# acproject/wsi-segmentation-pipeline

Hardware: AMD Instinct MI355X
Metric: patches/sec (256×256×3) whole-slide inference, 1/2/4/8 MI355X + CPU ref (higher is better)
Workload: dtype fp16 + MX-fp6 cross terms (fp32 accumulate); 1 GPU; cfg3: ONE 40000x40000 synthetic slide, tile 256 stride 256 -> 24648 tiles sharded over 1 rank(s) (each holds only its own slide regions: 4.80 GB on rank 0), ResNet-18 trunk + Classifier, fused read+normalise+conv HIP path, 1 all-gather, float64 stitch + softmax; tiles_total=24648, batch=6200, mode=mx, parallelism=tile-shard x1 + 1 all-gather, batches_in_flight=2

## Files before the change

### include/wsi_hip.h

```cpp
#ifndef WSI_HIP_H
#define WSI_HIP_H
#include <stddef.h>
#include <stdint.h>

#ifdef __cplusplus
extern "C" {
#endif

#define WSI_HIP_ABI_VERSION 8
int wsi_hip_abi_version(void);

size_t wsi_pf_bytes(int n, int h, int w, int c, int planes);
long long wsi_pf_pixel_index(int n, int y, int x, int h, int w);

size_t wsi_prepack_conv_bytes(int cout, int cin, int k, int planes);
int wsi_prepack_conv(const float* w, const float* bn_weight, const float* bn_bias, const float* bn_mean,
                     const float* bn_var, float eps, int cout, int cin, int k, int planes, void* wpk_out,
                     float* bias_out);
size_t wsi_prepack_stem_bytes(int planes);
int wsi_prepack_stem(const float* w, const float* bn_weight, const float* bn_bias, const float* bn_mean,
                     const float* bn_var, float eps, int planes, void* wpk_out, float* bias_out);
int wsi_prepack_stem_u8(const float* w, const float* bn_weight, const float* bn_bias, const float* bn_mean,
                        const float* bn_var, float eps, const float mean[3], const float std_[3], int planes,
                        void* wpk_out, float* bias_out);
// ... 6 lines not shown
                                     const float* stem_bias_u8, const float* norm_mean_std ,
                                     int n, int h, int w, float* scratch, void* out_pf, int planes, void* stream);

int wsi_stem_conv7x7_bn_relu_maxpool_lines96(const float* in_f32, const uint8_t* slide, long long slide_pitch_bytes,
                                             int slide_h, int slide_w, const int* tile_xy, const float* lut,
                                             const void* stem_wpk, const float* stem_bias, const void* stem_wpk_u8,
                                             const float* stem_bias_u8, const float* norm_mean_std, int n, int h, int w,
                                             float* scratch, void* out_pf96, long long plane96, void* stream);

enum {
    WSI_STEM_MODE_UNFUSED = 0,
    WSI_STEM_MODE_FUSED = 1,
    WSI_STEM_MODE_FUSED_LUT = 2,
    WSI_STEM_MODE_FUSED_ONE_STRIP = 3,
    WSI_STEM_MODE_FUSED_STRIPS = 4
};
int wsi_stem_set_mode(int fused, int rows_per_seg);

int wsi_conv3x3_bn_act(const void* in_pf, void* out_pf, const void* resid_pf, const void* wpk, const float* bias,
                       int n, int h_in, int w_in, int cin, int cout, int stride, int relu, int planes,
                       void* stream);
int wsi_conv1x1_bn(const void* in_pf, void* out_pf, const void* wpk, const float* bias, int n, int h_in, int w_in,
                   int cin, int cout, int stride, int planes, void* stream);
int wsi_conv3x3_up_concat_bn_act(const void* up_pf, const void* skip_pf, void* out_pf, const void* wpk, const float* bias, int n, int h, int w,
                                 int c_up, int c_skip, int cout, int relu, int planes, void* stream);
int wsi_conv3x3s2_ds_fused(const void* in_pf, void* out_conv_pf, void* out_ds_pf, const void* wpk3, const float* bias3,
                           const void* wpk1, const float* bias1, int n, int h_in, int w_in, int cin, int cout, int planes,
                           void* stream);
int wsi_s2_slab_images(int n, int h_in, int w_in, int cin, int planes);
size_t wsi_pf_split_bytes(int n, int h, int w, int c, int planes);
int wsi_conv3x3_bn_act_split(const void* in_pf, void* out_split, const void* resid_pf, const void* wpk, const float* bias,
                             int n, int h, int w, int cin, int cout, int relu, int planes, void* stream);
int wsi_conv3x3s2_ds_fused_split(const void* in_split, void* out_conv_pf, void* out_ds_pf, const void* wpk3,
                                 const float* bias3, const void* wpk1, const float* bias1, int n, int h_in, int w_in,
                                 int cin, int cout, int planes, void* stream);
enum {
    WSI_CONV_MODE_S2_GATHER = 0,
    WSI_CONV_MODE_S2_SLAB = 1,
    WSI_CONV_MODE_S2_SLAB_128 = 3,
    WSI_CONV_MODE_XCD_ORDER = 8,
    WSI_CONV_MODE_WIDE_FROM_256 = 16,
    WSI_CONV_MODE_WIDE_NEVER = 32,
    WSI_CONV_MODE_S2_ABLATE = 64,
    WSI_CONV_MODE_NO_S2_SPLIT = 128,
    WSI_CONV_MODE_XCD_RANGES_OFF = 256,
    WSI_CONV_MODE_XCD_RANGES_L1 = 512,
    WSI_CONV_MODE_L1_SLAB3 = 1024,
    WSI_CONV_MODE_NO_DS_FOLD = 2048,
    WSI_CONV_MODE_NO_SLAB_PAIR = 4096,
    WSI_CONV_MODE_L1_LINES128 = 16384,
    WSI_CONV_MODE_S2_NT2 = 32768,
    WSI_CONV_MODE_UNET_CONCAT_PASS = 65536,
    WSI_CONV_MODE_WIDE_NO_D8 = 131072,
    WSI_CONV_MODE_L1_PERSISTENT = 1048576,
    WSI_CONV_MODE_UNET_NO_TAIL = 2097152,
    WSI_CONV_MODE_UNET_TAIL_FORM1 = 4194304,
    WSI_CONV_MODE_UNET_X0_UNFUSED = 8388608
};
int wsi_conv_set_mode(int mode);
int wsi_conv3x3_bn_act_cfg(const void* in_pf, void* out_pf, const void* resid_pf, const void* wpk, const float* bias,
                           int n, int h_in, int w_in, int cin, int cout, int stride, int relu, int planes, int cfg,
                           void* stream);

int wsi_avgpool_fc(const void* in_pf, int n, int h, int w, int c, const float* fc_w, const float* fc_b, int k,
                   float* feat_out, float* logits_out, int planes, void* stream);
int wsi_linear(const float* x, const float* w, const float* bias, float* y, int b, int k, int j, int relu,
               void* stream);

int wsi_pf_pack(const float* in_nchw, void* out_pf, int n, int c, int h, int w, int planes, void* stream);
int wsi_pf_unpack(const void* in_pf, float* out_nchw, int n, int c, int h, int w, int planes, void* stream);

typedef struct {
    const void* stem_w;   const float* stem_b;
    const void* stem_w_u8; const float* stem_b_u8;
    float norm[6];
    const void* conv_w[16]; const float* conv_b[16];
    const void* down_w[3];  const float* down_b[3];
    const float* head_w;  const float* head_b;  int head_k;
    int planes;
} wsi_trunk_weights;

size_t wsi_trunk_workspace_bytes(int n, int h, int w, int planes);
int wsi_trunk_workspace_init(void* workspace, int n, int h, int w, int planes, void* stream);
int wsi_trunk_workspace_release(void* workspace);
int wsi_trunk_forward(const wsi_trunk_weights* wt, const float* in_f32, const uint8_t* slide,
                      long long slide_pitch_bytes, int slide_h, int slide_w, const int* tile_xy, const float* lut,
                      int n, int h, int w, void* workspace, int workspace_n, float* feat_out ,
                      float* logits_out , float* fmap_out ,
                      void* stream);
int wsi_trunk_set_chunks(int stem_chunk, int layer1_chunk);
int wsi_trunk_forward_tap(const wsi_trunk_weights* wt, const float* in_f32, const uint8_t* slide,
                          long long slide_pitch_bytes, int slide_h, int slide_w, const int* tile_xy, const float* lut,
                          int n, int h, int w, void* workspace, int workspace_n, int stop_after, float* tap_out_nchw,
                          void* stream);

int wsi_prof_begin(int max_records);
int wsi_prof_end(float* ms_out, int* kind_out, double* flops_out, int cap);

int wsi_tile_gather(const uint8_t* slide, long long slide_pitch_bytes, int slide_h, int slide_w, const int* tile_xy,
                    const float* lut, float* out_nchw, int n, int ph, int pw, void* stream);
int wsi_stitch_add(const float* tile_logits, const int* map_xy, int t, int c, int dy, int dx, double* pred, int map_h,
                   int map_w, void* stream);
int wsi_stitch_add_dense(const float* tile_pred, const int* map_xy, int t, int c, int ph, int pw, double* pred, int map_h,
                         int map_w, void* stream);
int wsi_softmax_threshold_argmax(const double* pred, int c, long long hw, const double* class_thresh, double* probs,
                                 uint8_t* classes, const uint8_t* mask, int heat_mode, uint8_t* heat, void* stream);
// ... 76 lines not shown
```

### wsi_segmentation_pipeline_amd/csrc/capi.hip

```cpp
#include "internal.h"
#include "../../include/wsi_hip.h"

ConvRoutes g_routes;

StemArgs stem_args(const TileSource& src, const void* wpk, const float* bias, float* scratch, int n, int h, int w) {
    StemArgs a;
    a.mode = src.in_f32 ? 0 : 1;
    a.in_f32 = src.in_f32; a.slide = src.slide; a.slide_pitch = src.pitch; a.SH = src.SH; a.SW = src.SW;
    a.origins = src.tile_xy; a.lut = src.lut; a.wpk = wpk; a.bias = bias; a.out = scratch;
    a.N = n; a.H = h; a.W = w; a.wpk_u8 = nullptr; a.bias_u8 = nullptr;
    return a;
}

int stem_run(const TileSource& src, const void* stem_wpk, const float* stem_bias, const void* stem_wpk_u8, const float* stem_bias_u8,
             const float* norm_mean_std, int n, int h, int w, float* scratch, void* out_pf, int planes, void* stream, int out96,
             long long plane96, void* x0_pf) {
    if (!stem_wpk || !stem_bias || !scratch || !out_pf || n <= 0 || h % 16 || w % 4) return WSI_EINVAL;
    if (!src.valid()) return WSI_EINVAL;
    StemArgs a = stem_args(src, stem_wpk, stem_bias, scratch, n, h, w);
    if (stem_wpk_u8 && stem_bias_u8 && norm_mean_std && !src.in_f32 && g_routes.stem_u8x) { a.wpk_u8 = stem_wpk_u8; a.bias_u8 = stem_bias_u8; }
    if (out96 && planes != 3) return WSI_EINVAL;
    if (x0_pf && !(a.wpk_u8 && g_routes.stem_fused && planes == 2)) return WSI_EINVAL;
    if (g_routes.stem_fused || planes == 3) return wsi_stem_pool_dispatch(a, out_pf, planes, g_routes.stem_rows, (hipStream_t)stream, out96, plane96, x0_pf);
    int rc = wsi_stem_dispatch(a, planes, (hipStream_t)stream);
// ... 171 lines not shown
    if (!fits(1)) return 0;
    int lo = 1, hi = n;
    while (hi - lo > 1) {
        const int mid = lo + (hi - lo) / 2;
        (fits(mid) ? lo : hi) = mid;
    }
    return lo;
}

int wsi_conv3x3s2_ds_fused(const void* in_pf, void* out_conv_pf, void* out_ds_pf, const void* wpk3, const float* bias3,
                           const void* wpk1, const float* bias1, int n, int h_in, int w_in, int cin, int cout, int planes,
                           void* stream) {
    if (!s2_ds_ok(in_pf, out_conv_pf, out_ds_pf, wpk3, bias3, wpk1, bias1, n, h_in, w_in, false)) return WSI_EINVAL;
    ConvArgs a = s2_ds_args(in_pf, out_conv_pf, out_ds_pf, wpk3, bias3, wpk1, bias1, n, h_in, w_in, cin, cout);
    const int per = wsi_s2_slab_images(n, h_in, w_in, cin, planes);
    const size_t bpc = planes == 1 ? PFmt<1>::BPC : PFmt<2>::BPC;
    const size_t in_img = (size_t)(h_in + 1) * (w_in + 1) * cin * bpc, out_img = (size_t)(h_in / 2 + 1) * (w_in / 2 + 1) * cout * bpc;
    int rc = WSI_EINVAL;
    for (int n0 = 0; per > 0 && n0 < n; n0 += per) {
        const int nn = n - n0 < per ? n - n0 : per;
        a.in = (const char*)in_pf + n0 * in_img;
        a.out = (char*)out_conv_pf + n0 * out_img;
        a.out2 = (char*)out_ds_pf + n0 * out_img;
        a.gi = pf_geom_fd(nn, h_in, w_in, cin);
        a.go = pf_geom_fd(nn, h_in / 2, w_in / 2, cout);
        rc = wsi_s2_dispatch(a, planes, (hipStream_t)stream);
        if (rc) break;
    }
    if (rc == WSI_EINVAL) {
        ConvCall c = {.in = in_pf, .out = out_conv_pf, .wpk = wpk3, .bias = bias3, .n = n, .h = h_in, .w = w_in, .cin = cin, .cout = cout,
                      .stride = 2, .ksize = 3, .relu = 1, .planes = planes, .stream = stream, .cfg = 0};
        rc = conv_common(c);
        c.out = out_ds_pf; c.wpk = wpk1; c.bias = bias1; c.ksize = 1; c.relu = 0;
        if (!rc) rc = conv_common(c);
    }
    return rc;
}

int wsi_conv_set_mode(int mode) {
    ConvRoutes& r = g_routes;
    const int base = mode & 7;
    r.s2_slab = base != WSI_CONV_MODE_S2_GATHER;
    r.s2_small_tiles = base != WSI_CONV_MODE_S2_SLAB_128;
    r.xcd_order = (mode & WSI_CONV_MODE_XCD_ORDER) ? 1 : 0;
    r.wide_min_c = (mode & WSI_CONV_MODE_WIDE_FROM_256) ? 256 : (mode & WSI_CONV_MODE_WIDE_NEVER) ? (1 << 30) : 128;
    r.s2_ablate = (mode & WSI_CONV_MODE_S2_ABLATE) ? 1 : 0;
    r.s2_split = (mode & WSI_CONV_MODE_NO_S2_SPLIT) ? 0 : 1;
    r.xcd_ranges = (mode & WSI_CONV_MODE_XCD_RANGES_OFF) ? 0 : (mode & WSI_CONV_MODE_XCD_RANGES_L1) ? 1 : 2;
    r.l1_rows = (mode & WSI_CONV_MODE_L1_SLAB3) ? 0 : 1;
    r.ds_fold = (mode & WSI_CONV_MODE_NO_DS_FOLD) ? 0 : 1;
    r.slab_pair = (mode & WSI_CONV_MODE_NO_SLAB_PAIR) ? 0 : 1;
    r.l1_lines96 = (mode & WSI_CONV_MODE_L1_LINES128) ? 0 : 1;
    r.s2_nt4 = (mode & WSI_CONV_MODE_S2_NT2) ? 0 : 1;
    r.unet_fuse_up = (mode & WSI_CONV_MODE_UNET_CONCAT_PASS) ? 0 : 1;
    r.wide_d8 = (mode & WSI_CONV_MODE_WIDE_NO_D8) ? 0 : 1;
    r.l1p = (mode & WSI_CONV_MODE_L1_PERSISTENT) ? 1 : 0;
    r.unet_tail = (mode & WSI_CONV_MODE_UNET_NO_TAIL) ? 0 : 1;
    r.unet_tail_form = (mode & WSI_CONV_MODE_UNET_TAIL_FORM1) ? 1 : 2;
    r.unet_x0_fused = (mode & WSI_CONV_MODE_UNET_X0_UNFUSED) ? 0 : 1;
    return WSI_OK;
}

int wsi_conv1x1_bn(const void* in_pf, void* out_pf, const void* wpk, const float* bias, int n, int h_in, int w_in,
                   int cin, int cout, int stride, int planes, void* stream) {
    return conv_common({.in = in_pf, .out = out_pf, .wpk = wpk, .bias = bias, .n = n, .h = h_in, .w = w_in, .cin = cin, .cout = cout,
                        .stride = stride, .ksize = 1, .relu = 0, .planes = planes, .stream = stream});
}

int wsi_avgpool_fc(const void* in_pf, int n, int h, int w, int c, const float* fc_w, const float* fc_b, int k,
                   float* feat_out, float* logits_out, int planes, void* stream) {
    if (!in_pf || n <= 0 || (logits_out && (!fc_w || !fc_b || k <= 0))) return WSI_EINVAL;
    return wsi_avgpool_fc_dispatch(in_pf, pf_geom(n, h, w, c), fc_w, fc_b, k, feat_out, logits_out, planes,
                                   (hipStream_t)stream);
}

int wsi_linear(const float* x, const float* w, const float* bias, float* y, int b, int k, int j, int relu,
               void* stream) {
    if (!x || !w || !y) return WSI_EINVAL;
    return wsi_linear_dispatch(x, w, bias, y, b, k, j, relu, (hipStream_t)stream);
}

int wsi_pf_pack(const float* in_nchw, void* out_pf, int n, int c, int h, int w, int planes, void* stream) {
    if (!in_nchw || !out_pf || n <= 0 || planes < 1 || planes > 3 || c % (planes == 1 ? 64 : 32)) return WSI_EINVAL;
    return wsi_pf_pack_dispatch(in_nchw, out_pf, pf_geom(n, h, w, c), planes, (hipStream_t)stream);
}

int wsi_pf_unpack(const void* in_pf, float* out_nchw, int n, int c, int h, int w, int planes, void* stream) {
    if (!in_pf || !out_nchw || n <= 0 || planes < 1 || planes > 3 || c % (planes == 1 ? 64 : 32)) return WSI_EINVAL;
    return wsi_pf_unpack_dispatch(in_pf, out_nchw, pf_geom(n, h, w, c), planes, (hipStream_t)stream);
}

int wsi_tile_gather(const uint8_t* slide, long long slide_pitch_bytes, int slide_h, int slide_w, const int* tile_xy,
                    const float* lut, float* out_nchw, int n, int ph, int pw, void* stream) {
    if (!slide || !tile_xy || !lut || !out_nchw) return WSI_EINVAL;
    return wsi_tile_gather_dispatch(slide, slide_pitch_bytes, slide_h, slide_w, tile_xy, lut, out_nchw, n, ph, pw,
                                    (hipStream_t)stream);
}

int wsi_stitch_add(const float* tile_logits, const int* map_xy, int t, int c, int dy, int dx, double* pred, int map_h,
                   int map_w, void* stream) {
    if (!tile_logits || !map_xy || !pred || map_h <= 0 || map_w <= 0) return WSI_EINVAL;
    return wsi_stitch_add_dispatch(tile_logits, map_xy, t, c, dy, dx, pred, map_h, map_w, (hipStream_t)stream);
}

int wsi_stitch_add_dense(const float* tile_pred, const int* map_xy, int t, int c, int ph, int pw, double* pred, int map_h,
                         int map_w, void* stream) {
// ... 126 lines not shown
```

### wsi_segmentation_pipeline_amd/csrc/common.h

```cpp
#pragma once
#include <hip/hip_runtime.h>
#include <stdint.h>

typedef __attribute__((ext_vector_type(8))) __bf16 bf16x8;
typedef __attribute__((ext_vector_type(4))) __bf16 bf16x4;
typedef __attribute__((ext_vector_type(16))) float f32x16;
typedef __attribute__((ext_vector_type(4))) float f32x4;

#define WSI_OK 0
#define WSI_EINVAL (-22)
#define WSI_ENOMEM (-12)
#define WSI_EFAULT (-14)

struct FastDiv { unsigned m; int s; };
static inline FastDiv fastdiv_make(int d) {
    FastDiv f;
    if (d <= 1) { f.m = 0u; f.s = -1; return f; }
    int l = 0;
    while ((1ll << l) < d) ++l;
    f.m = (unsigned)(((1ull << (31 + l)) / (unsigned long long)d) + 1ull);
    f.s = l - 1;
    return f;
}
#ifdef __HIPCC__
// ... 215 lines not shown
    lo = (_Float16)(x - (float)hi);
}
static inline __device__ void split_f16x4(const float* v, f16x4& hi, f16x4& lo) {
#pragma unroll
    for (int i = 0; i < 4; ++i) {
        _Float16 a, b;
        split_f16(v[i], a, b);
        hi[i] = a;
        lo[i] = b;
    }
}
static inline __device__ const float* conv_wscale_inv(const void* wpk, int cout, int cin, int ksize) {
    return (const float*)((const char*)wpk + (size_t)(cout / 32) * (cin / 32) * ksize * ksize * 4096);
}

struct StemArgs {
    int mode;
    const float* in_f32;
    const uint8_t* slide;
    long long slide_pitch;
    int SH, SW;
    const int* origins;
    const float* lut;
    const void* wpk;
    const float* bias;
    float* out;
    int N, H, W;
    const void* wpk_u8;
    const float* bias_u8;
    void* out_pf = nullptr;
    int out_planes = 0;
};

struct ConvRoutes {
    int stem_fused = 1;
    int stem_rows = 64;
    int stem_u8x = 1;
    int stem_shared_weights = 1;
    int stem_dense = 1;
    int chunk_stem = 0;
    int chunk_l1 = 0;
    int s2_slab = 1;
    int s2_small_tiles = 1;
    int xcd_order = 0;
    int wide_min_c = 128;
    int s2_ablate = 0;
    int s2_split = 1;
    int xcd_ranges = 2;
    int l1_rows = 1;
    int ds_fold = 1;
    int slab_pair = 1;
    int l1_lines96 = 1;
    int s2_nt4 = 1;
    int unet_fuse_up = 1;
    int wide_d8 = 1;
    int l1p = 0;
    int unet_tail = 1;
    int unet_tail_form = 2;
    int unet_x0_fused = 1;
};
extern ConvRoutes g_routes;
```

### wsi_segmentation_pipeline_amd/csrc/conv.hip

```cpp
#include "conv_dev.h"
#include "internal.h"

template <int MT, int WM, int WN, int PLANES>
__global__ __launch_bounds__(WM* WN * 64) void conv_gather_kernel(ConvArgs a) {
    extern __shared__ __attribute__((aligned(16))) char smem[];
    constexpr int BM = WM * MT * 32;
    constexpr int NTHREADS = WM * WN * 64;
    constexpr int PPT = BM * 8 / NTHREADS;
    constexpr int PIX_STEP = NTHREADS / 8;
    const int tid = threadIdx.x, lane = tid & 63, wave = tid >> 6;
    const int wm = wave / WN, wn = wave % WN;
    const int l31 = lane & 31, h = lane >> 5;
    const int nblocks = a.go.C / (WN * 32);
    const int nb = blockIdx.x % nblocks;
    const int mtile = blockIdx.x / nblocks;
    const int q0 = a.go.G + mtile * BM;
    const int ntile = nb * WN + wn;
    const int NC = a.gi.C / PFmt<PLANES>::CPL;
    const int KS = a.ksize, NT = KS * KS, pad = KS / 2;
    const size_t in_pixstride = (size_t)a.gi.C * PFmt<PLANES>::BPC;
    const bf16x8* wbase = (const bf16x8*)a.wpk + (size_t)ntile * NC * NT * 4 * 64 + lane;

    int inq[PPT];
    const int sp = tid & 7;
// ... 1083 lines not shown
                else if (c + 1 < NC) wload(wbuf[0], c + 1, 0);
            }
            asm volatile("" ::: "memory");
            const int toff = tap_off(t, Pc);
            const int toff_next = t + 1 < NT ? tap_off(t + 1, Pc) : 0;
#pragma unroll
            for (int mt = 0; mt < MT; ++mt) {
                const int k = t * MT + mt;
                if (mt + 1 < MT) xload(xf[(k + 1) & 1], xoff[mt + 1] + toff);
                else if (t + 1 < NT) xload(xf[(k + 1) & 1], xoff[0] + toff_next);
                const bf16x8(&w)[4] = wbuf[t % RING];
                const bf16x8(&x)[4] = xf[k & 1];
                f32x16& d = (FUSE && t == 9) ? accd[FUSE ? mt : 0] : acc[mt];
                if constexpr (PLANES == 3) {
                    d = mfma_mx6(d, w, x);
                } else if constexpr (PLANES == 2) {
                    mfma_step<2>(d, w, x);
                } else {
#pragma unroll
                    for (int f = 0; f < 4; ++f) d = mfma_bf16(w[f], x[f], d);
                }
            }
        }
    }
    conv_epilogue_any<MT, PLANES>(a, acc, q0 + wm * MT * 32, ntile, lane);
    if constexpr (FUSE) {
        ConvArgs a2 = a;
        a2.out = a.out2; a2.bias = a.bias2; a2.resid = nullptr; a2.relu = 0;
        a2.wpk = a.wpk2; a2.ksize = 1;
        conv_epilogue_any<MT, PLANES>(a2, accd, q0 + wm * MT * 32, ntile, lane);
    }
}

template <int MT, int WM, int WN, int PLANES, int MINW, bool FUSE, int PMAX = 34, int ABL = 0>
static int launch_s2slab(const ConvArgs& a, hipStream_t st) {
    constexpr int BM = WM * MT * 32, NTHREADS = WM * WN * 64;
    if (a.go.C % (WN * 32) || a.go.P > PMAX) return WSI_EINVAL;
    if ((unsigned long long)pf_alloc_pixels(a.gi.N, a.gi.H, a.gi.W) * a.gi.C * PFmt<PLANES>::BPC >= 0xffffffffull) return WSI_EINVAL;
    const int mtiles = (a.go.NS + BM - 1) / BM;
    const int nblocks = a.go.C / (WN * 32);
    const int npieces = (4 * BM + 2 * a.go.P + 2) * 8;
    const size_t lds = (size_t)((npieces + NTHREADS - 1) / NTHREADS * NTHREADS) * 16;
    if (lds > 160 * 1024) return WSI_EINVAL;
    auto k = conv3x3s2_slab_kernel<MT, WM, WN, PLANES, MINW, FUSE, PMAX, ABL>;
    if (lds > 64 * 1024) {
        if (hipFuncSetAttribute((const void*)k, hipFuncAttributeMaxDynamicSharedMemorySize, (int)lds) != hipSuccess)
            return WSI_EINVAL;
    }
    const int grid = (a.flags & CONV_XCD_ORDER) ? (mtiles + 7) / 8 * 8 * nblocks : mtiles * nblocks;
    hipLaunchKernelGGL(k, dim3(grid), dim3(NTHREADS), lds, st, a);
    return hipGetLastError() == hipSuccess ? WSI_OK : WSI_EFAULT;
}

template <int PLANES, bool DENSE, bool DS, int NT = 2>
__global__ __launch_bounds__(512, 1) void conv3x3s2_wide_kernel(ConvArgs a) {
    extern __shared__ __attribute__((aligned(16))) char smem[];
    static_assert(NT == 2 || (NT == 4 && !DS), "four channel tiles per wave: no second accumulator set");
    constexpr int MT = 2, BM = 256, NTILES = 2 * NT, ULEN = NT == 2 ? 2 : 1;
    constexpr int WBUF = NTILES * 4096, XB = 45056;
    constexpr int NWB = 2 * ULEN;
    char* const wl = smem;
    char* const xl0 = smem + NWB * WBUF;
    const int tid = threadIdx.x, lane = tid & 63;
    const int wave = __builtin_amdgcn_readfirstlane(tid >> 6);
    const int wm = wave >> 1, wn = wave & 1;
    const int l31 = lane & 31, h = lane >> 5;
    const int nblocks = a.go.C / (NTILES * 32);
    const int chunk = gridDim.x >> 3, lin = (blockIdx.x & 7) * chunk + (blockIdx.x >> 3);
    const int nb = lin % nblocks, mtile = lin / nblocks;
    if (mtile >= a.mtiles) return;
    const int P = a.go.P;
    int q0, qlast, qs[MT];
    bool valid[MT];
    if constexpr (!DENSE) {
        q0 = a.go.G + mtile * BM;
        qlast = q0 + BM - 1;
#pragma unroll
        for (int mt = 0; mt < MT; ++mt) {
            qs[mt] = q0 + wm * MT * 32 + mt * 32 + l31;
            valid[mt] = pf_is_pixel(a.go, qs[mt]);
        }
    } else {
        const int HW = a.go.H * a.go.W, R = a.go.N * HW;
        auto pos = [&](int i) { return pf_pos_of_index(a.go, i); };
        const int i0 = mtile * BM, i1 = min(i0 + BM, R) - 1;
        q0 = pos(i0);
        qlast = pos(i1);
#pragma unroll
        for (int mt = 0; mt < MT; ++mt) {
            const int i = i0 + wm * MT * 32 + mt * 32 + (a.go.W < 32 ? dense_lane_pixel(l31) : l31);
            valid[mt] = i < R;
            qs[mt] = pos(valid[mt] ? i : i1);
        }
    }
    const int NC = a.gi.C / PFmt<PLANES>::CPL;
    const size_t in_pixstride = (size_t)a.gi.C * PFmt<PLANES>::BPC;
    const __amdgpu_buffer_rsrc_t wrs = __builtin_amdgcn_make_buffer_rsrc(
        (void*)((const char*)a.wpk + (size_t)(nb * NTILES) * NC * 9 * 4096), 0, NTILES * NC * 9 * 4096, 0x00020000);
    const __amdgpu_buffer_rsrc_t wrd = __builtin_amdgcn_make_buffer_rsrc(
        (void*)((const char*)(DS ? a.wpk2 : a.wpk) + (size_t)(nb * NTILES) * NC * 4096), 0, NTILES * NC * 4096, 0x00020000);
    const int wvoff = lane * 16;
    auto wdma = [&](int c, int t, char* wb) {
#pragma unroll
        for (int j = 0; j < NTILES; ++j) {
            if (t < 9) dma16_buf_asm(wrs, lds_addr_of(wb) + j * 4096 + (wave - 4) * 1024, wvoff, ((j * NC + c) * 9 + t) * 4096 + (wave - 4) * 1024);
            else dma16_buf_asm(wrd, lds_addr_of(wb) + j * 4096 + (wave - 4) * 1024, wvoff, (j * NC + c) * 4096 + (wave - 4) * 1024);
        }
    };
    auto xdma = [&](int c, int ph, char* xb) {
        const int back = ((ph & 2) ? P : 0) + (ph & 1);
        const char* src = (const char*)a.in + ((size_t)ph * a.in_split_pixels + (size_t)(q0 - back)) * in_pixstride + c * 128;
        const int npieces = (qlast - q0 + 1 + back) * 8;
        for (int i0 = wave * 64; i0 < npieces; i0 += 256) {
            const int i = i0 + lane;
            const int Pl = i >> 3, sl = (i & 7) ^ ((Pl >> 1) & 7);
            dma16_asm(src + (size_t)Pl * in_pixstride + sl * 16, lds_addr_of(xb) + i0 * 16);
        }
    };
    auto wread = [&](bf16x8(&w)[NT][4], const char* wb) {
        const char* src = wb + (wn * NT) * 4096 + lane * 16;
#pragma unroll
        for (int nt = 0; nt < NT; ++nt) {
#pragma unroll
            for (int f = 0; f < 4; ++f) w[nt][f] = *(const bf16x8*)(src + nt * 4096 + f * 1024);
        }
    };

    f32x16 acc[NT][MT], accd[DS ? NT : 1][DS ? MT : 1];
#pragma unroll
    for (int nt = 0; nt < NT; ++nt) {
        if constexpr (PLANES == 3) {
            acc_init_bias<MT>(acc[nt], a.bias, nb * NTILES + wn * NT + nt, lane);
            if constexpr (DS) acc_init_bias<MT>(accd[nt], a.bias2, nb * NTILES + wn * NT + nt, lane);
        } else {
#pragma unroll
            for (int mt = 0; mt < MT; ++mt)
#pragma unroll
                for (int r = 0; r < 16; ++r) {
                    acc[nt][mt][r] = 0.f;
                    if constexpr (DS) accd[nt][mt][r] = 0.f;
                }
        }
    }

    constexpr int SPL = DS ? 10 : 9;
    constexpr int STEP_TAP[10] = {4, DS ? 9 : 3, DS ? 3 : 5, DS ? 5 : 1, DS ? 1 : 7, DS ? 7 : 0, DS ? 0 : 2, DS ? 2 : 6, DS ? 6 : 8, 8};
    constexpr int UNIT0[4] = {0, DS ? 2 : 1, DS ? 4 : 3, DS ? 6 : 5};
    constexpr int NSTEP[4] = {DS ? 2 : 1, 2, 2, 4};
    const int NG = NC * SPL;
    auto wdma_step = [&](int c, int j) {
        const int cc = c + j / SPL, g = cc * SPL + j % SPL;
        if (g < NG) wdma(cc, STEP_TAP[j % SPL], wl + (g & (NWB - 1)) * WBUF);
    };
    if (wave < 4) xdma(0, 0, xl0);
    else { wdma_step(0, 0); if (NSTEP[0] == 2 && ULEN == 2) wdma_step(0, 1); }
    asm volatile("s_waitcnt vmcnt(0)" ::: "memory");
    __syncthreads();
    for (int c = 0; c < NC; ++c) {
#pragma unroll
        for (int ph = 0; ph < 4; ++ph) {
            const char* xl = xl0 + (size_t)(ph & 1) * XB;
            if (wave < 4) {
                if (ph < 3) xdma(c, ph + 1, xl0 + (size_t)((ph + 1) & 1) * XB);
                else if (c + 1 < NC) xdma(c + 1, 0, xl0);
            }
#pragma unroll
            for (int kp = 0; kp < NSTEP[ph]; kp += ULEN) {
                const int j0 = UNIT0[ph] + kp;
                const int ulen = NSTEP[ph] - kp >= ULEN ? ULEN : 1;
                const int jn = j0 + ulen;
                const int nlen = ULEN == 1 ? 1 : (kp + 2 < NSTEP[ph]) ? 2 : (ph < 3 ? (NSTEP[ph + 1] >= 2 ? 2 : 1) : (NSTEP[0] >= 2 ? 2 : 1));
                if (wave >= 4) { wdma_step(c, jn); if (nlen == 2) wdma_step(c, jn + 1); }
#pragma unroll
                for (int k = 0; k < ulen; ++k) {
                    const int g = c * SPL + j0 + k;
                    const int t = STEP_TAP[j0 + k];
                    constexpr bool PREF = NT == 2 && !DS;
                    bf16x8 wf[NT][4], xf[PREF ? 2 : MT][4];
                    wread(wf, wl + (g & (NWB - 1)) * WBUF);
                    const int sh = (t < 9 && t % 3 == 2 ? 1 : 0) + (t < 9 && t / 3 == 2 ? P : 0);
                    auto xload = [&](bf16x8(&x)[4], int mt) {
                        int ql = qs[mt] - q0;
                        asm volatile("" : "+v"(ql));
                        const int Pl = ql + sh;
                        const int base = lds_xbase(Pl, h);
#pragma unroll
                        for (int f = 0; f < 4; ++f) x[f] = *(const bf16x8*)(xl + (base ^ (f << 5)));
                    };
                    if constexpr (PREF) {
                        xload(xf[0], 0);
#pragma unroll
                        for (int mt = 0; mt < MT; ++mt) {
                            if (mt + 1 < MT) xload(xf[(mt + 1) & 1], mt + 1);
                            __builtin_amdgcn_sched_barrier(0);
#pragma unroll
                            for (int nt = 0; nt < NT; ++nt) mfma_step<PLANES>(acc[nt][mt], wf[nt], xf[mt & 1]);
                            __builtin_amdgcn_sched_barrier(0);
                        }
                    } else {
#pragma unroll
                        for (int mt = 0; mt < MT; ++mt) xload(xf[mt], mt);
#pragma unroll
                        for (int mt = 0; mt < MT; ++mt)
#pragma unroll
                            for (int nt = 0; nt < NT; ++nt) {
                                if constexpr (DS) mfma_step<PLANES>(t == 9 ? accd[nt][mt] : acc[nt][mt], wf[nt], xf[mt]);
                                else mfma_step<PLANES>(acc[nt][mt], wf[nt], xf[mt]);
                            }
                    }
                }
                if (wave >= 4 || kp + ULEN >= NSTEP[ph]) asm volatile("s_waitcnt vmcnt(0)" ::: "memory");
                __syncthreads();
            }
        }
    }
#pragma unroll
    for (int nt = 0; nt < NT; ++nt) {
        const int ntile = nb * NTILES + wn * NT + nt;
        if constexpr (PLANES == 3) {
            conv_epilogue_mx<MT>(a, acc[nt], qs, valid, ntile, lane);
        } else {
            conv_epilogue_q<MT, PLANES>(a, acc[nt], qs, valid, ntile, lane);
        }
        if constexpr (DS) {
            ConvArgs a2 = a;
            a2.out = a.out2; a2.bias = a.bias2; a2.resid = nullptr; a2.relu = 0;
            a2.wpk = a.wpk2; a2.ksize = 1;
            if constexpr (PLANES == 3) conv_epilogue_mx<MT>(a2, accd[nt], qs, valid, ntile, lane);
            else conv_epilogue_q<MT, PLANES>(a2, accd[nt], qs, valid, ntile, lane);
        }
    }
}

template <int PLANES>
static int launch_s2wide(const ConvArgs& a, hipStream_t st) {
    constexpr int BM = 256, XB = 45056;
    const bool ds = a.out2 != nullptr;
    if (a.go.C % 128 || a.go.P > 34 || !a.in_split_pixels || (ds && (!a.wpk2 || !a.bias2)) || a.out_split_pixels) return WSI_EINVAL;
    const long long R = (long long)a.go.N * a.go.H * a.go.W;
    const bool nt4 = !ds && PLANES == 3 && g_routes.s2_nt4 && a.go.C % 256 == 0;
    const int nblocks = a.go.C / (nt4 ? 256 : 128);
    ConvArgs g = a;
    g.gi = a.go;
    const long long span = dense_max_slab_pixels(g, BM) - (a.go.P + 1);
    const bool dense = (span * 8 + 255) / 256 * 256 * 16 <= XB;
    const int mtiles = dense ? (int)((R + BM - 1) / BM) : (a.go.NS + BM - 1) / BM;
    const size_t lds = 4 * 16384 + 2 * XB;
    auto k = nt4 ? (dense ? conv3x3s2_wide_kernel<PLANES, true, false, 4> : conv3x3s2_wide_kernel<PLANES, false, false, 4>)
           : dense ? (ds ? conv3x3s2_wide_kernel<PLANES, true, true> : conv3x3s2_wide_kernel<PLANES, true, false>)
                   : (ds ? conv3x3s2_wide_kernel<PLANES, false, true> : conv3x3s2_wide_kernel<PLANES, false, false>);
    if (hipFuncSetAttribute((const void*)k, hipFuncAttributeMaxDynamicSharedMemorySize, (int)lds) != hipSuccess) return WSI_EINVAL;
    ConvArgs b = a;
    b.mtiles = mtiles;
    hipLaunchKernelGGL(k, dim3((mtiles * nblocks + 7) / 8 * 8), dim3(512), lds, st, b);
    return hipGetLastError() == hipSuccess ? WSI_OK : WSI_EFAULT;
}

int wsi_s2_dispatch(const ConvArgs& a_in, int planes, hipStream_t st) {
    ConvArgs a = a_in;
    if (a.in_split_pixels)
        return planes == 3 ? launch_s2wide<3>(a, st) : planes == 2 ? launch_s2wide<2>(a, st) : WSI_EINVAL;
    if (g_routes.xcd_order && a.go.C > 128) a.flags |= CONV_XCD_ORDER;
    if (a.gi.C % 64 || a.go.C % 128 || planes < 1 || planes > 3) return WSI_EINVAL;
    if (a.go.H * 2 != a.gi.H || a.go.W * 2 != a.gi.W || a.gi.N != a.go.N) return WSI_EINVAL;
    const bool fuse = a.out2 != nullptr;
    if (fuse && (!a.wpk2 || !a.bias2)) return WSI_EINVAL;
    if (a.go.P > 34) {
        if (planes == 3) return fuse ? launch_s2slab<2, 1, 4, 3, 2, true, 130>(a, st) : launch_s2slab<2, 1, 4, 3, 2, false, 130>(a, st);
        if (planes == 2) return fuse ? launch_s2slab<2, 1, 4, 2, 2, true, 130>(a, st) : launch_s2slab<2, 1, 4, 2, 2, false, 130>(a, st);
        return WSI_EINVAL;
    }
#ifdef WSI_STUDY
    if (g_routes.s2_ablate && planes == 3 && fuse) return launch_s2slab<2, 1, 4, 3, 3, true, 34, 16>(a, st);
#endif
    if (g_routes.s2_small_tiles) {
        if (planes == 3) return fuse ? launch_s2slab<2, 1, 4, 3, 3, true>(a, st) : launch_s2slab<2, 1, 4, 3, 3, false>(a, st);
        if (planes == 2) return fuse ? launch_s2slab<2, 1, 4, 2, 3, true>(a, st) : launch_s2slab<2, 1, 4, 2, 3, false>(a, st);
    }
    if (planes == 3) return fuse ? launch_s2slab<4, 1, 4, 3, 2, true>(a, st) : launch_s2slab<4, 1, 4, 3, 2, false>(a, st);
    if (planes == 2) return fuse ? launch_s2slab<4, 1, 4, 2, 2, true>(a, st) : launch_s2slab<4, 1, 4, 2, 2, false>(a, st);
    return fuse ? launch_s2slab<4, 1, 4, 1, 2, true>(a, st) : launch_s2slab<4, 1, 4, 1, 2, false>(a, st);
}

template <int MT, int WM, int WN, int PLANES>
static int launch_gather(const ConvArgs& a, hipStream_t st) {
    constexpr int BM = WM * MT * 32;
    if (a.go.C % (WN * 32)) return WSI_EINVAL;
    const int mtiles = (a.go.NS + BM - 1) / BM;
    const int nblocks = a.go.C / (WN * 32);
    const size_t lds = (size_t)BM * 128;
    hipLaunchKernelGGL((conv_gather_kernel<MT, WM, WN, PLANES>), dim3(mtiles * nblocks), dim3(WM * WN * 64), lds, st, a);
    return hipGetLastError() == hipSuccess ? WSI_OK : WSI_EFAULT;
}

#define SLAB3_CFGS(X) \
    X(20, 4, 1, 4, 2, false) \
    X(21, 4, 2, 2, 2, false) \
    X(25, 2, 2, 4, 3, false) \
    X(27, 4, 4, 2, 1, false) \
    X(28, 2, 2, 2, 3, true) \
    X(29, 2, 2, 2, 4, true) \
    X(39, 4, 4, 2, 1, true) \
    X(26, 4, 1, 2, 3, false) \
    X(30, 4, 1, 4, 2, true) \
    X(31, 4, 2, 2, 2, true) \
    X(32, 2, 2, 4, 3, true) \
    X(33, 8, 1, 4, 2, true) \
// ... 90 lines not shown
```

### wsi_segmentation_pipeline_amd/native.py

```python
import contextlib
import ctypes as C
import enum
import os
import subprocess

_HERE = os.path.dirname(os.path.abspath(__file__))
LIB_PATH = os.path.join(_HERE, 'lib', 'libwsi_hip.so')
CSRC = os.path.join(_HERE, 'csrc')

_lib = None


class NativeLibraryMissing(RuntimeError):
    pass


class WsiTrunkWeights(C.Structure):
    _fields_ = [
        ('stem_w', C.c_void_p), ('stem_b', C.c_void_p),
        ('stem_w_u8', C.c_void_p), ('stem_b_u8', C.c_void_p), ('norm', C.c_float * 6),
        ('conv_w', C.c_void_p * 16), ('conv_b', C.c_void_p * 16),
        ('down_w', C.c_void_p * 3), ('down_b', C.c_void_p * 3),
        ('head_w', C.c_void_p), ('head_b', C.c_void_p), ('head_k', C.c_int),
        ('planes', C.c_int),
# ... 100 lines not shown


def build(verbose=False):
    res = subprocess.run(['make', '-C', CSRC, '-j8'], stdout=subprocess.PIPE, stderr=subprocess.STDOUT, text=True)
    if verbose or res.returncode:
        print(res.stdout)
    if res.returncode:
        raise RuntimeError('hipcc build of libwsi_hip.so failed')
    global _lib
    _lib = None
    return LIB_PATH


ABI_VERSION = 8


def load():
    global _lib
    if _lib is not None:
        return _lib
    if not os.path.exists(LIB_PATH):
        raise NativeLibraryMissing(
            '%s not found: the WSI inference path has no CPU fallback - build it first '
            '(python -c "import __graft_entry__ as g; g.build()" or make -C %s)' % (LIB_PATH, CSRC))
    lib = C.CDLL(LIB_PATH)
    for name, (res, args) in SIGNATURES.items():
        fn = getattr(lib, name)
        fn.restype = res
        fn.argtypes = args
    if lib.wsi_hip_abi_version() != ABI_VERSION:
        raise RuntimeError('libwsi_hip.so ABI version mismatch')
    _lib = lib
    return lib


class ConvMode(enum.IntFlag):
    S2_GATHER = 0
    S2_SLAB = 1
    S2_SLAB_128 = 3
    XCD_ORDER = 8
    WIDE_FROM_256 = 16
    WIDE_NEVER = 32
    S2_ABLATE = 64
    NO_S2_SPLIT = 128
    XCD_RANGES_OFF = 256
    XCD_RANGES_L1 = 512
    L1_SLAB3 = 1024
    NO_DS_FOLD = 2048
    NO_SLAB_PAIR = 4096
    L1_LINES128 = 16384
    S2_NT2 = 32768
    UNET_CONCAT_PASS = 65536
    WIDE_NO_D8 = 131072
    L1_PERSISTENT = 1048576
    UNET_NO_TAIL = 2097152
    UNET_TAIL_FORM1 = 4194304
    UNET_X0_UNFUSED = 8388608


class StemMode(enum.IntEnum):
    UNFUSED = 0
    FUSED = 1
    FUSED_LUT = 2
    FUSED_ONE_STRIP = 3
    FUSED_STRIPS = 4


@contextlib.contextmanager
def conv_mode(flags=0, base=ConvMode.S2_SLAB):
    lib = load()
    check(lib.wsi_conv_set_mode(int(base) | int(flags)), 'wsi_conv_set_mode')
    try:
        yield
    finally:
        lib.wsi_conv_set_mode(int(ConvMode.S2_SLAB))


@contextlib.contextmanager
def stem_mode(fused, rows=64):
    lib = load()
    check(lib.wsi_stem_set_mode(int(fused), rows), 'wsi_stem_set_mode')
    try:
        yield
    finally:
        lib.wsi_stem_set_mode(int(StemMode.FUSED), 64)


def check(rc, what):
    if rc != 0:
        raise RuntimeError('%s failed with code %d (see include/wsi_hip.h error conventions)' % (what, rc))
```

Baseline: 121,600 patches/s.

## Add four-wave two-workgroup-per-CU form of stride-2 wide conv kernel

Adds a 256-thread variant of the stride-2 wide conv kernel with a single input buffer and half the LDS, launch-bounded for two workgroups per CU. It is used by default for 3-plane, non-downsample layers that do not take the NT4 route. The aim is to overlap two workgroups per CU in place of double-buffering inside one. In exchange, each input phase load now waits with an extra barrier, and fewer waves issue the weight DMA.

```diff
diff --git a/include/wsi_hip.h b/include/wsi_hip.h
--- a/include/wsi_hip.h
+++ b/include/wsi_hip.h
@@ -82,6 +82,7 @@
     WSI_CONV_MODE_S2_NT2 = 32768,
     WSI_CONV_MODE_UNET_CONCAT_PASS = 65536,
     WSI_CONV_MODE_WIDE_NO_D8 = 131072,
+    WSI_CONV_MODE_S2_8WAVE = 262144,
     WSI_CONV_MODE_L1_PERSISTENT = 1048576,
     WSI_CONV_MODE_UNET_NO_TAIL = 2097152,
     WSI_CONV_MODE_UNET_TAIL_FORM1 = 4194304,
diff --git a/wsi_segmentation_pipeline_amd/csrc/capi.hip b/wsi_segmentation_pipeline_amd/csrc/capi.hip
--- a/wsi_segmentation_pipeline_amd/csrc/capi.hip
+++ b/wsi_segmentation_pipeline_amd/csrc/capi.hip
@@ -247,6 +247,7 @@
     r.slab_pair = (mode & WSI_CONV_MODE_NO_SLAB_PAIR) ? 0 : 1;
     r.l1_lines96 = (mode & WSI_CONV_MODE_L1_LINES128) ? 0 : 1;
     r.s2_nt4 = (mode & WSI_CONV_MODE_S2_NT2) ? 0 : 1;
+    r.s2_w4 = (mode & WSI_CONV_MODE_S2_8WAVE) ? 0 : 1;
     r.unet_fuse_up = (mode & WSI_CONV_MODE_UNET_CONCAT_PASS) ? 0 : 1;
     r.wide_d8 = (mode & WSI_CONV_MODE_WIDE_NO_D8) ? 0 : 1;
     r.l1p = (mode & WSI_CONV_MODE_L1_PERSISTENT) ? 1 : 0;
diff --git a/wsi_segmentation_pipeline_amd/csrc/common.h b/wsi_segmentation_pipeline_amd/csrc/common.h
--- a/wsi_segmentation_pipeline_amd/csrc/common.h
+++ b/wsi_segmentation_pipeline_amd/csrc/common.h
@@ -291,6 +291,7 @@
     int slab_pair = 1;
     int l1_lines96 = 1;
     int s2_nt4 = 1;
+    int s2_w4 = 1;
     int unet_fuse_up = 1;
     int wide_d8 = 1;
     int l1p = 0;
diff --git a/wsi_segmentation_pipeline_amd/csrc/conv.hip b/wsi_segmentation_pipeline_amd/csrc/conv.hip
--- a/wsi_segmentation_pipeline_amd/csrc/conv.hip
+++ b/wsi_segmentation_pipeline_amd/csrc/conv.hip
@@ -1159,18 +1159,22 @@
     return hipGetLastError() == hipSuccess ? WSI_OK : WSI_EFAULT;
 }
 
-template <int PLANES, bool DENSE, bool DS, int NT = 2>
-__global__ __launch_bounds__(512, 1) void conv3x3s2_wide_kernel(ConvArgs a) {
+template <int PLANES, bool DENSE, bool DS, int NT = 2, bool W4 = false>
+__global__ __launch_bounds__(W4 ? 256 : 512, W4 ? 2 : 1) void conv3x3s2_wide_kernel(ConvArgs a) {
     extern __shared__ __attribute__((aligned(16))) char smem[];
     static_assert(NT == 2 || (NT == 4 && !DS), "four channel tiles per wave: no second accumulator set");
-    constexpr int MT = 2, BM = 256, NTILES = 2 * NT, ULEN = NT == 2 ? 2 : 1;
+    constexpr int PW = W4 ? 2 : 4;
+    constexpr int WNC = W4 ? 1 : 2;
+    constexpr int XBUFS = W4 ? 1 : 2;
+    constexpr int MT = 2, BM = 256, NTILES = WNC * NT, ULEN = NT == 2 ? 2 : 1;
+    static_assert(!W4 || NTILES == 4, "four-wave form: 128 couts per workgroup");
     constexpr int WBUF = NTILES * 4096, XB = 45056;
     constexpr int NWB = 2 * ULEN;
     char* const wl = smem;
     char* const xl0 = smem + NWB * WBUF;
     const int tid = threadIdx.x, lane = tid & 63;
     const int wave = __builtin_amdgcn_readfirstlane(tid >> 6);
-    const int wm = wave >> 1, wn = wave & 1;
+    const int wm = wave / WNC, wn = wave % WNC;
     const int l31 = lane & 31, h = lane >> 5;
     const int nblocks = a.go.C / (NTILES * 32);
     const int chunk = gridDim.x >> 3, lin = (blockIdx.x & 7) * chunk + (blockIdx.x >> 3);
@@ -1210,19 +1214,23 @@
     auto wdma = [&](int c, int t, char* wb) {
 #pragma unroll
         for (int j = 0; j < NTILES; ++j) {
-            if (t < 9) dma16_buf_asm(wrs, lds_addr_of(wb) + j * 4096 + (wave - 4) * 1024, wvoff, ((j * NC + c) * 9 + t) * 4096 + (wave - 4) * 1024);
-            else dma16_buf_asm(wrd, lds_addr_of(wb) + j * 4096 + (wave - 4) * 1024, wvoff, (j * NC + c) * 4096 + (wave - 4) * 1024);
+#pragma unroll
+            for (int r = 0; r < 4 / PW; ++r) {
+                const int part = ((wave - PW) * (4 / PW) + r) * 1024;
+                if (t < 9) dma16_buf_asm(wrs, lds_addr_of(wb) + j * 4096 + part, wvoff, ((j * NC + c) * 9 + t) * 4096 + part);
+                else dma16_buf_asm(wrd, lds_addr_of(wb) + j * 4096 + part, wvoff, (j * NC + c) * 4096 + part);
+            }
         }
     };
     auto xdma = [&](int c, int ph, char* xb) {
         const int back = ((ph & 2) ? P : 0) + (ph & 1);
         const char* src = (const char*)a.in + ((size_t)ph * a.in_split_pixels + (size_t)(q0 - back)) * in_pixstride + c * 128;
         const int npieces = (qlast - q0 + 1 + back) * 8;
-        for (int i0 = wave * 64; i0 < npieces; i0 += 256) {
-            const int i = i0 + lane;
-            const int Pl = i >> 3, sl = (i & 7) ^ ((Pl >> 1) & 7);
-            dma16_asm(src + (size_t)Pl * in_pixstride + sl * 16, lds_addr_of(xb) + i0 * 16);
-        }
+        const int i = wave * 64 + lane, Pl = i >> 3, sl = (i & 7) ^ ((Pl >> 1) & 7);
+        const char* p = src + (size_t)Pl * in_pixstride + sl * 16;
+        const size_t dp = (size_t)32 * in_pixstride;
+        unsigned l = lds_addr_of(xb) + wave * 1024;
+        for (int i0 = wave * 64; i0 < npieces; i0 += 256, p += dp, l += 4096) dma16_asm(p, l);
     };
     auto wread = [&](bf16x8(&w)[NT][4], const char* wb) {
         const char* src = wb + (wn * NT) * 4096 + lane * 16;
@@ -1259,15 +1267,15 @@
         const int cc = c + j / SPL, g = cc * SPL + j % SPL;
         if (g < NG) wdma(cc, STEP_TAP[j % SPL], wl + (g & (NWB - 1)) * WBUF);
     };
-    if (wave < 4) xdma(0, 0, xl0);
-    else { wdma_step(0, 0); if (NSTEP[0] == 2 && ULEN == 2) wdma_step(0, 1); }
+    if (XBUFS == 1 || wave < PW) xdma(0, 0, xl0);
+    if (wave >= PW) { wdma_step(0, 0); if (NSTEP[0] == 2 && ULEN == 2) wdma_step(0, 1); }
     asm volatile("s_waitcnt vmcnt(0)" ::: "memory");
     __syncthreads();
     for (int c = 0; c < NC; ++c) {
 #pragma unroll
         for (int ph = 0; ph < 4; ++ph) {
-            const char* xl = xl0 + (size_t)(ph & 1) * XB;
-            if (wave < 4) {
+            const char* xl = xl0 + (size_t)(ph & (XBUFS - 1)) * XB;
+            if (XBUFS == 2 && wave < PW) {
                 if (ph < 3) xdma(c, ph + 1, xl0 + (size_t)((ph + 1) & 1) * XB);
                 else if (c + 1 < NC) xdma(c + 1, 0, xl0);
             }
@@ -1277,7 +1285,7 @@
                 const int ulen = NSTEP[ph] - kp >= ULEN ? ULEN : 1;
                 const int jn = j0 + ulen;
                 const int nlen = ULEN == 1 ? 1 : (kp + 2 < NSTEP[ph]) ? 2 : (ph < 3 ? (NSTEP[ph + 1] >= 2 ? 2 : 1) : (NSTEP[0] >= 2 ? 2 : 1));
-                if (wave >= 4) { wdma_step(c, jn); if (nlen == 2) wdma_step(c, jn + 1); }
+                if (wave >= PW) { wdma_step(c, jn); if (nlen == 2) wdma_step(c, jn + 1); }
 #pragma unroll
                 for (int k = 0; k < ulen; ++k) {
                     const int g = c * SPL + j0 + k;
@@ -1316,7 +1324,13 @@
                             }
                     }
                 }
-                if (wave >= 4 || kp + ULEN >= NSTEP[ph]) asm volatile("s_waitcnt vmcnt(0)" ::: "memory");
+                if (wave >= PW || (XBUFS == 2 && kp + ULEN >= NSTEP[ph])) asm volatile("s_waitcnt vmcnt(0)" ::: "memory");
+                __syncthreads();
+            }
+            if constexpr (XBUFS == 1) {
+                if (ph < 3) xdma(c, ph + 1, xl0);
+                else if (c + 1 < NC) xdma(c + 1, 0, xl0);
+                asm volatile("s_waitcnt vmcnt(0)" ::: "memory");
                 __syncthreads();
             }
         }
@@ -1346,20 +1360,24 @@
     if (a.go.C % 128 || a.go.P > 34 || !a.in_split_pixels || (ds && (!a.wpk2 || !a.bias2)) || a.out_split_pixels) return WSI_EINVAL;
     const long long R = (long long)a.go.N * a.go.H * a.go.W;
     const bool nt4 = !ds && PLANES == 3 && g_routes.s2_nt4 && a.go.C % 256 == 0;
+    const bool w4 = !ds && PLANES == 3 && !nt4 && g_routes.s2_w4;
     const int nblocks = a.go.C / (nt4 ? 256 : 128);
     ConvArgs g = a;
     g.gi = a.go;
     const long long span = dense_max_slab_pixels(g, BM) - (a.go.P + 1);
     const bool dense = (span * 8 + 255) / 256 * 256 * 16 <= XB;
     const int mtiles = dense ? (int)((R + BM - 1) / BM) : (a.go.NS + BM - 1) / BM;
-    const size_t lds = 4 * 16384 + 2 * XB;
-    auto k = nt4 ? (dense ? conv3x3s2_wide_kernel<PLANES, true, false, 4> : conv3x3s2_wide_kernel<PLANES, false, false, 4>)
+    const size_t lds = w4 ? 2 * 16384 + XB : 4 * 16384 + 2 * XB;
+    void (*k)(ConvArgs) = nt4 ? (dense ? conv3x3s2_wide_kernel<PLANES, true, false, 4> : conv3x3s2_wide_kernel<PLANES, false, false, 4>)
            : dense ? (ds ? conv3x3s2_wide_kernel<PLANES, true, true> : conv3x3s2_wide_kernel<PLANES, true, false>)
                    : (ds ? conv3x3s2_wide_kernel<PLANES, false, true> : conv3x3s2_wide_kernel<PLANES, false, false>);
+    if constexpr (PLANES == 3) {
+        if (w4) k = dense ? conv3x3s2_wide_kernel<3, true, false, 4, true> : conv3x3s2_wide_kernel<3, false, false, 4, true>;
+    }
     if (hipFuncSetAttribute((const void*)k, hipFuncAttributeMaxDynamicSharedMemorySize, (int)lds) != hipSuccess) return WSI_EINVAL;
     ConvArgs b = a;
     b.mtiles = mtiles;
-    hipLaunchKernelGGL(k, dim3((mtiles * nblocks + 7) / 8 * 8), dim3(512), lds, st, b);
+    hipLaunchKernelGGL(k, dim3((mtiles * nblocks + 7) / 8 * 8), dim3(w4 ? 256 : 512), lds, st, b);
     return hipGetLastError() == hipSuccess ? WSI_OK : WSI_EFAULT;
 }
 
diff --git a/wsi_segmentation_pipeline_amd/native.py b/wsi_segmentation_pipeline_amd/native.py
--- a/wsi_segmentation_pipeline_amd/native.py
+++ b/wsi_segmentation_pipeline_amd/native.py
@@ -176,6 +176,7 @@
     S2_NT2 = 32768
     UNET_CONCAT_PASS = 65536
     WIDE_NO_D8 = 131072
+    S2_8WAVE = 262144
     L1_PERSISTENT = 1048576
     UNET_NO_TAIL = 2097152
     UNET_TAIL_FORM1 = 4194304
```

Measured after the change: 122,900 patches/s, median of 6. 1.0% higher.
